# penn-graphics-research/HOT

Measured on AMD Instinct MI355X. Metric: ms per nonlinear (L-BFGS) iteration; P2G+G2P Mparticles/s; achieved HBM GB/s vs roofline, lower is better.
Workload: dtype f64; 1 GPU; C2: one 63^3-cell cube x 8 ppc (63^3 cells per GPU), fixed-corotated E=50000 nu=0.3, dx=0.01, dt=1/24, -lsolver 3 -mg_level 3 -smoother 5 -coarseSolver 2 --project --linesearch --bcproject --usecn -cneps 1e-7; particles_per_gpu=2000376, particles_total=2000376, nodes_total=267562, levels=3, parallelism=1 GPU

## Files before the change

### hot_amd/csrc/hot_common.h

```cpp
#pragma once
#include <hip/hip_runtime.h>
#include <cstdint>
#include <cstdio>
#include <cstring>
#include <cstdlib>
#include <string>
#include <vector>
#include <map>
#include <chrono>
#include "../../include/hot_mi355x.h"

namespace hot {

struct Error {
    int code;
    std::string msg;
};

#define HOT_HIP(expr)                                                                                             \
    do {                                                                                                          \
        hipError_t _e = (expr);                                                                                   \
        if (_e != hipSuccess) throw ::hot::Error{ HOT_ERR_DEVICE, std::string(#expr) + ": " + hipGetErrorString(_e) }; \
    } while (0)

// ... 109 lines not shown
    T d1 = d0 - (T)1;
    w[1] = (T)0.75 - d1 * d1;
    T d2 = (T)1 - d1;
    T zz = (T)1.5 - d2;
    w[2] = (T)0.5 * zz * zz;
    dw[0] = -z;
    dw[1] = -(T)2 * d1;
    dw[2] = zz;
}

template <int CTRL, int ROW_MASK>
__device__ __forceinline__ float dpp_move(float v)
{
    return __int_as_float(__builtin_amdgcn_update_dpp(0, __float_as_int(v), CTRL, ROW_MASK, 0xf, false));
}
template <int CTRL, int ROW_MASK>
__device__ __forceinline__ double dpp_move(double v)
{
    long long b = __double_as_longlong(v);
    int lo = __builtin_amdgcn_update_dpp(0, (int)(b & 0xffffffffLL), CTRL, ROW_MASK, 0xf, false);
    int hi = __builtin_amdgcn_update_dpp(0, (int)(b >> 32), CTRL, ROW_MASK, 0xf, false);
    return __longlong_as_double(((long long)hi << 32) | (unsigned int)lo);
}
__device__ __forceinline__ float wave_last(float v) { return __int_as_float(__builtin_amdgcn_readlane(__float_as_int(v), 63)); }
__device__ __forceinline__ double wave_last(double v)
{
    long long b = __double_as_longlong(v);
    int lo = __builtin_amdgcn_readlane((int)(b & 0xffffffffLL), 63), hi = __builtin_amdgcn_readlane((int)(b >> 32), 63);
    return __longlong_as_double(((long long)hi << 32) | (unsigned int)lo);
}
template <class T>
__device__ inline T wave_sum(T v)
{
    v += dpp_move<0xb1, 0xf>(v);
    v += dpp_move<0x4e, 0xf>(v);
    v += dpp_move<0x114, 0xf>(v);
    v += dpp_move<0x118, 0xf>(v);
    v += dpp_move<0x142, 0xa>(v);
    v += dpp_move<0x143, 0xc>(v);
    return wave_last(v);
}
template <class T>
__device__ inline T block_sum_256(T v, T* sm4)
{
    v = wave_sum(v);
    int lane = threadIdx.x & 63, w = threadIdx.x >> 6;
// ... 211 lines not shown
```

### hot_amd/csrc/mg_gs.hip

```cpp
#include "hot_impl.h"

namespace hot {

#ifdef HOT_AB_KERNELS
#include "ab_src/mg_gs_ab1.hip"
#endif

template <class T, int SB>
struct GsLds {
    static constexpr int TRI = SB * (SB - 1) / 2 + 1;
    static constexpr size_t bytes = (size_t)9 * TRI * sizeof(T) + SB * 3 * sizeof(T) + 5 * SB * sizeof(int32_t);
};
template <class T>
struct GsWinv {
    static constexpr int img_elems = (9 * GsLds<T, 64>::TRI + 15) / 16 * 16;
};
template <int SB>
__device__ __forceinline__ int gs_tri_fwd(int row, int colm) { return (SB - 1) * colm - (colm * (colm - 1)) / 2 + (row - colm - 1); }
__device__ __forceinline__ int gs_tri_bwd(int row, int colm) { return (colm * (colm - 1)) / 2 + row; }
template <bool FWD>
__device__ __forceinline__ int gs_winv_idx(int row, int colm) { return FWD ? (row * (row - 1)) / 2 + colm : ((63 - row) * (62 - row)) / 2 + (63 - colm); }

template <class T>
__device__ __forceinline__ void gs_store_tri(T* tri, int TRI, int idx, const T* __restrict__ di, const T (&b)[9])
// ... 678 lines not shown
__device__ unsigned long long gs_clk[34 * 8];
#define GS_CLK(i) \
    do { \
        const unsigned long long t_ = clock64(); \
        gclk_[i] += t_ - gt0_, gt0_ = t_; \
    } while (0)
#else
#define GS_CLK(i)
#endif
template <class T, bool FWD, int SB, bool WINV = false>
__global__ __launch_bounds__(SB * 16) void k_gs_sweep(const int32_t* __restrict__ col, const T* __restrict__ val, const uint32_t* __restrict__ ckey, const int32_t* __restrict__ gs_order,
    const int32_t* __restrict__ block_start, const T* __restrict__ diagVal, const T* __restrict__ diagBlockInv, const T* __restrict__ rhs, T* x, T* hD, GsPasses P,
    const int32_t* __restrict__ rowcnt, int* done, int* err, const int32_t* __restrict__ nbr, int* flag, int epoch, int dataflag,
    T* unset_next ,
    const T* __restrict__ gs_w )
{
    extern __shared__ __attribute__((aligned(16))) char gs_smem[];
    constexpr int TRI = GsLds<T, SB>::TRI;
    static_assert(!WINV || SB == 64, "the inverse images are whole-block images");
#ifdef HOT_GS_CLOCKS
    unsigned long long gclk_[5] = { 0, 0, 0, 0, 0 }, gt0_ = clock64();
#endif
    constexpr int RQ = 4, NW = SB / RQ;
    auto ld3 = [&](int64_t j, T& x0, T& x1, T& x2) {
        x0 = __hip_atomic_load(x + 3 * j, __ATOMIC_RELAXED, __HIP_MEMORY_SCOPE_AGENT), x1 = __hip_atomic_load(x + 3 * j + 1, __ATOMIC_RELAXED, __HIP_MEMORY_SCOPE_AGENT),
        x2 = __hip_atomic_load(x + 3 * j + 2, __ATOMIC_RELAXED, __HIP_MEMORY_SCOPE_AGENT);
        if (!dataflag) return;
        int spins = 0;
        while (GsUnset<T>::is(x0) || GsUnset<T>::is(x1) || GsUnset<T>::is(x2)) {
            __builtin_amdgcn_s_sleep(2);
            if (++spins > (1 << 21) || ((spins & 1023) == 0 && *(volatile int*)err)) {
                *(volatile int*)err = 1;
                break;
            }
            x0 = __hip_atomic_load(x + 3 * j, __ATOMIC_RELAXED, __HIP_MEMORY_SCOPE_AGENT), x1 = __hip_atomic_load(x + 3 * j + 1, __ATOMIC_RELAXED, __HIP_MEMORY_SCOPE_AGENT),
            x2 = __hip_atomic_load(x + 3 * j + 2, __ATOMIC_RELAXED, __HIP_MEMORY_SCOPE_AGENT);
        }
    };
    T* tri = (T*)gs_smem;
    T* sv = tri + (WINV ? GsWinv<T>::img_elems : 9 * TRI);
    int32_t* nodes = (int32_t*)(sv + 3 * SB);
    const int tid = threadIdx.x, lane = tid & 63, w = tid >> 6;
    int p = 0;
    while (p + 1 < P.npass && (int)blockIdx.x >= P.wg_begin[p + 1]) ++p;
    const int b = P.block0[p] + ((int)blockIdx.x - P.wg_begin[p]);
    const int lo = P.sub[p] * SB;
    const int start = block_start[b] + lo, cnt = max(0, min(SB, block_start[b + 1] - start));
    T* sDinv = (T*)(nodes + 5 * SB);
    T* sD = sDinv + 9 * SB;
    T* srhs = sD + 9 * SB;
    if (!WINV)
        for (int e = tid; e < 9 * TRI; e += 64 * NW) tri[e] = (T)0;
    if (tid < SB) nodes[tid] = tid < cnt ? gs_order[start + tid] : -1;
    __syncthreads();
    GS_CLK(0);
    if (WINV) {
        constexpr int IMG_BYTES = GsWinv<T>::img_elems * (int)sizeof(T);
        const char* wg = (const char*)(gs_w + ((size_t)b * 2 + (FWD ? 0 : 1)) * GsWinv<T>::img_elems);
        for (int c = w; c * 1024 < IMG_BYTES; c += NW) {
            const int off = c * 1024 + lane * 16;
            if (off < IMG_BYTES)
                __builtin_amdgcn_global_load_lds((const __attribute__((address_space(1))) void*)(wg + off), (__attribute__((address_space(3))) void*)((char*)tri + c * 1024), 16, 0, 0);
        }
    }
    for (int e = tid; e < 9 * cnt; e += 64 * NW) {
        const int64_t i = nodes[e / 9];
        sDinv[e] = diagBlockInv[9 * i + e % 9];
        if (FWD) sD[e] = diagVal[9 * i + e % 9];
    }
    for (int e = tid; e < 3 * cnt; e += 64 * NW) srhs[e] = rhs[3 * (int64_t)nodes[e / 3] + e % 3];
    if (unset_next)
        for (int e = tid; e < 3 * cnt; e += 64 * NW) gs_store_unset(unset_next + 3 * (int64_t)nodes[e / 3] + e % 3);
    T bv[RQ][9];
    int jj[RQ], node[RQ], kb2[RQ], ke[RQ];
    const bool first_sub = p == 0 || P.color[p - 1] != P.color[p];
    const bool head = FWD ? first_sub : !first_sub;
    bool late[RQ];
    const uint32_t prevkey = p > 0 ? ((uint32_t)P.color[p - 1] << 8) | (uint32_t)P.sub[p - 1] : 0xffffffffu;
    if constexpr (WINV) {
        int4 rc[RQ];
#pragma unroll
        for (int q = 0; q < RQ; ++q) {
            const int ii = w + NW * q;
            jj[q] = -1, kb2[q] = 0, ke[q] = 0, late[q] = false;
            node[q] = ii < cnt ? nodes[ii] : -1;
#pragma unroll
            for (int e = 0; e < 9; ++e) bv[q][e] = (T)0;
        }
#pragma unroll
        for (int q = 0; q < RQ; ++q) rc[q] = node[q] >= 0 ? *(const int4*)(rowcnt + 4 * (int64_t)node[q]) : make_int4(0, 0, 0, 0);
#pragma unroll
        for (int q = 0; q < RQ; ++q) {
            if (node[q] < 0) continue;
            const int64_t i = node[q];
            const int kbeg = FWD ? 0 : rc[q].x + rc[q].y + 1 + rc[q].z, kend = FWD ? rc[q].x : kbeg + rc[q].w;
            kb2[q] = head ? kbeg + 64 : kbeg, ke[q] = head ? kend : kend - 64;
            const int k = head ? kbeg + lane : kend - 64 + lane;
            if (k >= kbeg && k < kend) {
                jj[q] = col[i * 125 + k];
                const T* bb = val + (i * 125 + k) * 9;
#pragma unroll
                for (int e = 0; e < 9; ++e) bv[q][e] = bb[e];
            }
        }
#pragma unroll
        for (int q = 0; q < RQ; ++q)
            if (jj[q] >= 0) {
                const uint32_t keyj = ckey[jj[q]];
                late[q] = (((keyj >> 28) << 8) | (((keyj & 127u) - 1u) / (uint32_t)SB)) == prevkey;
            }
    }
    else
#pragma unroll
    for (int q = 0; q < RQ; ++q) {
        const int ii = w + NW * q;
        jj[q] = -1, node[q] = -1, kb2[q] = 0, ke[q] = 0, late[q] = false;
#pragma unroll
        for (int e = 0; e < 9; ++e) bv[q][e] = (T)0;
        if (ii < cnt) {
            const int i = nodes[ii];
            node[q] = i;
            const int po = rowcnt[4 * i], pi = rowcnt[4 * i + 1], fi = rowcnt[4 * i + 2], fo = rowcnt[4 * i + 3];
            const int kbeg = FWD ? 0 : po + pi + 1, kend = FWD ? po + pi : po + pi + 1 + fi + fo;
            const int ibeg = FWD ? po : kbeg, iend = FWD ? po + pi : kbeg + fi;
            kb2[q] = head ? kbeg + 64 : kbeg, ke[q] = head ? kend : kend - 64;
            const int k = head ? kbeg + lane : kend - 64 + lane;
            if (k >= kbeg && k < kend) {
                const int j = col[(int64_t)i * 125 + k];
                const T* bb = val + ((int64_t)i * 125 + k) * 9;
#pragma unroll
                for (int e = 0; e < 9; ++e) bv[q][e] = bb[e];
                jj[q] = j;
                const uint32_t keyj = ckey[j];
                late[q] = (((keyj >> 28) << 8) | (((keyj & 127u) - 1u) / (uint32_t)SB)) == prevkey;
                if (k >= ibeg && k < iend) {
                    const int l = (int)(keyj & 127u) - 1 - lo;
                    if (l >= 0 && l < SB) {
                        if (!WINV) {
                            const int idx = FWD ? gs_tri_fwd<SB>(ii, l) : gs_tri_bwd(ii, l);
                            gs_store_tri<T>(tri, TRI, idx, diagBlockInv + 9 * (int64_t)i, bv[q]);
                        }
                        jj[q] = -1;
                    }
                }
            }
        }
    }
    int early_idx = -1, late_idx = -1;
    if (nbr && tid < 26) {
        const int nb = nbr[(int64_t)b * 26 + tid];
        if (nb >= 0) {
            const int cn = nb >> 28, gid = nb & 0x0fffffff;
            int qlast = -1;
            for (int q = 0; q < P.npass; ++q)
                if (P.color[q] == cn) qlast = q;
            if (qlast >= 0 && qlast < p) {
                if (qlast < p - 1)
                    early_idx = 4 * gid + P.sub[qlast];
                else {
                    late_idx = 4 * gid + P.sub[qlast];
                    if (qlast > 0 && P.color[qlast - 1] == cn) early_idx = 4 * gid + P.sub[qlast - 1];
                }
            }
        }
    }
    if (nbr && tid == 26 && p > 0 && P.color[p - 1] == P.color[p]) late_idx = 4 * b + P.sub[p - 1];
    if (nbr && tid == 27 && p > 1 && P.color[p - 2] == P.color[p]) early_idx = 4 * b + P.sub[p - 2];
    auto wait_blocks = [&](int idx) {
        if (idx < 0) return;
        int spins = 0;
        while (__hip_atomic_load(flag + idx, __ATOMIC_RELAXED, __HIP_MEMORY_SCOPE_AGENT) != epoch) {
            __builtin_amdgcn_s_sleep(4);
            if (++spins > (1 << 22) || ((spins & 1023) == 0 && *(volatile int*)err)) {
                *(volatile int*)err = 1;
                break;
            }
        }
    };
    if (dataflag) {
    }
    else if (nbr)
        wait_blocks(early_idx);
    else if (p > 1 && tid == 0) {
        const int need2 = P.wg_begin[p - 1] - P.wg_begin[p - 2];
        int spins = 0;
        while (__hip_atomic_load(done + p - 2, __ATOMIC_RELAXED, __HIP_MEMORY_SCOPE_AGENT) < need2) {
            __builtin_amdgcn_s_sleep(4);
            if (++spins > (1 << 22) || ((spins & 1023) == 0 && *(volatile int*)err)) {
                *(volatile int*)err = 1;
                break;
            }
        }
    }
    __syncthreads();
    GS_CLK(1);
    auto is_late = [&](uint32_t keyj) { return (((keyj >> 28) << 8) | (((keyj & 127u) - 1u) / (uint32_t)SB)) == prevkey; };
    bool tail_late[RQ];
#pragma unroll
    for (int q = 0; q < RQ; ++q) {
        const int ii = w + NW * q;
        tail_late[q] = false;
        if (ii >= cnt) continue;
        const int i = node[q];
        T e0 = 0, e1 = 0, e2 = 0;
        if (jj[q] >= 0 && !late[q]) {
            const int64_t j = jj[q];
            T x0, x1, x2;
            ld3(j, x0, x1, x2);
            e0 = bv[q][0] * x0 + bv[q][3] * x1 + bv[q][6] * x2;
            e1 = bv[q][1] * x0 + bv[q][4] * x1 + bv[q][7] * x2;
            e2 = bv[q][2] * x0 + bv[q][5] * x1 + bv[q][8] * x2;
        }
        bool tl = false;
        for (int k = kb2[q] + lane; k < ke[q]; k += 64) {
            const int j = col[(int64_t)i * 125 + k];
            const T* bb = val + ((int64_t)i * 125 + k) * 9;
            const uint32_t keyj = ckey[j], keyi = ckey[i];
            const int l = (int)(keyj & 127u) - 1 - lo;
            if ((keyj >> 7) == (keyi >> 7) && l >= 0 && l < SB) {
                if (!WINV) {
                    const int idx = FWD ? gs_tri_fwd<SB>(ii, l) : gs_tri_bwd(ii, l);
                    T bt[9];
#pragma unroll
                    for (int e = 0; e < 9; ++e) bt[e] = bb[e];
                    gs_store_tri<T>(tri, TRI, idx, diagBlockInv + 9 * (int64_t)i, bt);
                }
            }
            else if (is_late(keyj))
                tl = true;
            else {
                T x0, x1, x2;
                ld3(j, x0, x1, x2);
                e0 += bb[0] * x0 + bb[3] * x1 + bb[6] * x2;
                e1 += bb[1] * x0 + bb[4] * x1 + bb[7] * x2;
                e2 += bb[2] * x0 + bb[5] * x1 + bb[8] * x2;
            }
        }
        tail_late[q] = __ballot(tl) != 0ull;
        e0 = wave_sum(e0), e1 = wave_sum(e1), e2 = wave_sum(e2);
        if (lane == 0) srhs[3 * ii] -= e0, srhs[3 * ii + 1] -= e1, srhs[3 * ii + 2] -= e2;
    }
    GS_CLK(2);
    if (!dataflag) {
        if (nbr)
            wait_blocks(late_idx);
        else if (p > 0 && tid == 0) {
            const int need = P.wg_begin[p] - P.wg_begin[p - 1];
            int spins = 0;
            while (__hip_atomic_load(done + p - 1, __ATOMIC_RELAXED, __HIP_MEMORY_SCOPE_AGENT) < need) {
                __builtin_amdgcn_s_sleep(4);
                ++spins;
                if ((spins & 1023) == 0 && *(volatile int*)err) break;
                if (spins > (1 << 22)) {
                    *(volatile int*)err = 1;
                    break;
                }
            }
        }
        __syncthreads();
    }
#pragma unroll
    for (int q = 0; q < RQ; ++q) {
        const int ii = w + NW * q;
        if (ii >= cnt) continue;
        const int i = node[q];
        T s0 = 0, s1 = 0, s2 = 0;
        if (jj[q] >= 0 && late[q]) {
            const int64_t j = jj[q];
            T x0, x1, x2;
            ld3(j, x0, x1, x2);
            s0 = bv[q][0] * x0 + bv[q][3] * x1 + bv[q][6] * x2;
            s1 = bv[q][1] * x0 + bv[q][4] * x1 + bv[q][7] * x2;
            s2 = bv[q][2] * x0 + bv[q][5] * x1 + bv[q][8] * x2;
        }
        if (tail_late[q]) {
            for (int k = kb2[q] + lane; k < ke[q]; k += 64) {
                const int j = col[(int64_t)i * 125 + k];
                const T* bb = val + ((int64_t)i * 125 + k) * 9;
                const uint32_t keyj = ckey[j], keyi = ckey[i];
                const int l = (int)(keyj & 127u) - 1 - lo;
                if (!((keyj >> 7) == (keyi >> 7) && l >= 0 && l < SB) && is_late(keyj)) {
                    T x0, x1, x2;
                    ld3(j, x0, x1, x2);
                    s0 += bb[0] * x0 + bb[3] * x1 + bb[6] * x2;
                    s1 += bb[1] * x0 + bb[4] * x1 + bb[7] * x2;
                    s2 += bb[2] * x0 + bb[5] * x1 + bb[8] * x2;
                }
            }
        }
        s0 = wave_sum(s0), s1 = wave_sum(s1), s2 = wave_sum(s2);
        if (lane == 0) gs_store_rhs<T>(sv, ii, sDinv + 9 * ii, srhs[3 * ii] - s0, srhs[3 * ii + 1] - s1, srhs[3 * ii + 2] - s2);
    }
    __syncthreads();
    GS_CLK(3);
#ifdef HOT_GS_CLOCKS
#define GS_CLK_OUT() \
    do { \
        GS_CLK(4); \
        if (tid == 0) \
// ... 19 lines not shown
            T t0 = Lw[0] * ac0 + Lw[3] * ac1 + Lw[6] * ac2, t1 = Lw[1] * ac0 + Lw[4] * ac1 + Lw[7] * ac2, t2 = Lw[2] * ac0 + Lw[5] * ac1 + Lw[8] * ac2;
            t0 = wave_sum(t0), t1 = wave_sum(t1), t2 = wave_sum(t2);
            if (lane == k) h0 = sv[3 * rr] + t0, h1 = sv[3 * rr + 1] + t1, h2 = sv[3 * rr + 2] + t2;
        }
        const int me = 4 * w + lane;
        if (lane < 4 && me < cnt) {
            const int64_t i = nodes[me];
            __hip_atomic_store(x + 3 * i, h0, __ATOMIC_RELAXED, __HIP_MEMORY_SCOPE_AGENT);
            __hip_atomic_store(x + 3 * i + 1, h1, __ATOMIC_RELAXED, __HIP_MEMORY_SCOPE_AGENT);
            __hip_atomic_store(x + 3 * i + 2, h2, __ATOMIC_RELAXED, __HIP_MEMORY_SCOPE_AGENT);
            if (FWD) {
                const T* dd = sD + 9 * me;
                hD[3 * i] = dd[0] * h0 + dd[3] * h1 + dd[6] * h2, hD[3 * i + 1] = dd[1] * h0 + dd[4] * h1 + dd[7] * h2, hD[3 * i + 2] = dd[2] * h0 + dd[5] * h1 + dd[8] * h2;
            }
            else if (hD)
                hD[3 * i] += h0, hD[3 * i + 1] += h1, hD[3 * i + 2] += h2;
        }
        GS_CLK_OUT();
        return;
    }
    if (w != 0) return;
    if (cnt > 0) gs_phase_b<T, FWD, SB, true>(tri, sv, nodes, cnt, lane, diagVal, diagBlockInv, x, hD, sD);
    GS_CLK_OUT();
    if (dataflag) return;
    asm volatile("s_waitcnt vmcnt(0)" ::: "memory");
    if (lane == 0) {
        if (nbr)
            __hip_atomic_store(flag + 4 * b + P.sub[p], epoch, __ATOMIC_RELAXED, __HIP_MEMORY_SCOPE_AGENT);
        else
            __hip_atomic_fetch_add(done + p, 1, __ATOMIC_RELAXED, __HIP_MEMORY_SCOPE_AGENT);
    }
}

template <class T>
__global__ void k_gs_hdiff(size_t n3, T* __restrict__ h, const T* __restrict__ du)
{
    const size_t i = (size_t)blockIdx.x * blockDim.x + threadIdx.x;
    if (i < n3) h[i] -= du[i];
}
template <class T, bool DIFF = false>
__global__ __launch_bounds__(256) void k_gs_residual(const int32_t* __restrict__ col, const T* __restrict__ val, const int32_t* __restrict__ rowcnt, const T* __restrict__ h,
    const T* __restrict__ du, T* __restrict__ r, int n, const uint8_t* __restrict__ own, const uint8_t* __restrict__ owner ,
    int me, const T* __restrict__ l1e )
{
    const int lane = threadIdx.x & 63;
    const int row = xcd_block() * 4 + (threadIdx.x >> 6);
    if (row >= n || (own && !own[row])) return;
// ... 335 lines not shown
        gs_done.reserve(64);
    }
    bool du_marked = false;
    auto chained_sweep = [&](bool fwd) {
        const GsPasses& P = fwd ? PF : PB;
        if (P.npass == 0) return;
        const char* nm = fwd ? "gs_forward" : "gs_backward";
        const T* rhs = fwd ? r : dAu;
        T* xx = fwd ? hdu : du;
        T* hD = fwd ? dAu : u;
        const int32_t* rc = L.rowcnt.p;
        const bool marked = fwd ? tmp_marked : du_marked;
        if (fwd) tmp_marked = false;
        if (plan.dataflag && !marked)
            HOT_LAUNCH(this, "gs_fill_unset", k_gs_fill_unset<T>, div_up(n3, 256), 256, 0, n3, xx);
        else if (plan.dataflag)
            ;
        else if (plan.p2p)
            ++gs_epoch;
        else
            HOT_HIP(hipMemsetAsync(gs_done.p, 0, 40 * sizeof(int), stream));
        const int grid = P.wg_begin[P.npass];
        const int dataflag = plan.dataflag ? 1 : 0;
#define HOT_GS_CASE(F, S, ...)                                                                                                                                         \
    HOT_LAUNCH(this, lname(nm, L.id).c_str(), (k_gs_sweep<T, F, S, ##__VA_ARGS__>), grid, 16 * S, (GsLds<T, S>::bytes + 21 * S * sizeof(T) + 128), L.col.p, L.val.p, L.ckey.p, L.gs_order.p, L.gs_block_start.p, \
        L.diagVal.p, L.diagBlockInv.p, rhs, xx, hD, P, rc, gs_done.p, (int*)(hscal + 250), plan.p2p ? L.gs_nbr.p : (const int32_t*)nullptr, L.gs_flag.p, gs_epoch, dataflag, \
        (fwd && dataflag) ? du : (T*)nullptr, L.gs_w.p)
        du_marked = fwd && dataflag;
        if (plan.winv) {
            if (fwd)
                HOT_GS_CASE(true, 64, true);
            else
                HOT_GS_CASE(false, 64, true);
        }
        else if (fwd) {
            if (sb == 64) HOT_GS_CASE(true, 64);
            else if (sb == 32) HOT_GS_CASE(true, 32);
            else HOT_GS_CASE(true, 16);
        }
        else {
            if (sb == 64) HOT_GS_CASE(false, 64);
            else if (sb == 32) HOT_GS_CASE(false, 32);
            else HOT_GS_CASE(false, 16);
        }
#undef HOT_GS_CASE
    };
// ... 83 lines not shown
```

### hot_amd/csrc/mg_solve.hip

```cpp
#include "hot_impl.h"
#include "hot_svd.h"

namespace hot {

template <class T>
__global__ void k_axpy(size_t n, T a, const T* __restrict__ x, T* y)
{
    size_t i = (size_t)blockIdx.x * blockDim.x + threadIdx.x;
    if (i < n) y[i] += a * x[i];
}
template <class T>
__global__ void k_axpy_dev(size_t n, const double* a, double sign, const T* __restrict__ x, T* y)
{
    size_t i = (size_t)blockIdx.x * blockDim.x + threadIdx.x;
    T s = (T)(sign * (*a));
    if (i < n) y[i] += s * x[i];
}
template <class T>
__global__ void k_xpay_dev(size_t n, const double* a, const T* __restrict__ x, T* y)
{
    size_t i = (size_t)blockIdx.x * blockDim.x + threadIdx.x;
    T s = (T)(*a);
    if (i < n) y[i] = x[i] + s * y[i];
}
// ... 200 lines not shown
template <class T>
__global__ void k_cg_direction(size_t n3, const T* __restrict__ z, T* __restrict__ du, double* s, double* hm, double* ticket, double ticket_val)
{
    const size_t i = (size_t)blockIdx.x * blockDim.x + threadIdx.x;
    const bool act = cg_active(s[0], s[8]);
    if (act && i < n3) du[i] = z[i] + (T)(s[4] / s[0]) * du[i];
    if (i == 0) {
        if (act) {
            s[6] = 1.0;
            const double cnt = s[9] + 1.0;
            s[9] = cnt;
            hm[0] = s[4], hm[1] = cnt;
        }
        if (ticket) host_ticket_store(ticket, ticket_val);
    }
}
template <class T, int RPW = 0>
__global__ __launch_bounds__(1024) void k_cg_persist(const int32_t* __restrict__ col, const T* __restrict__ val, const T* __restrict__ Dinv, const T* __restrict__ init, T* __restrict__ u,
    T* __restrict__ r, T* __restrict__ z, T* du, T* __restrict__ dAu, int n, int max_iters, unsigned phase0 , double* dep , int SS , double* hm, double* ticket, double ticket_val,
    int* err )
{
    __shared__ double red[32], sres[2];
    __shared__ int s_bail;
    const int tid = threadIdx.x, lane = tid & 63, w = tid >> 6;
    const int G = gridDim.x, wg = blockIdx.x;
    unsigned phase = phase0;
    if (tid == 0) s_bail = 0;
    auto ldu = [&](int64_t j, int c) { return __hip_atomic_load(du + 3 * j + c, __ATOMIC_RELAXED, __HIP_MEMORY_SCOPE_AGENT); };
    auto sdu = [&](int64_t j, int c, T v) { __hip_atomic_store(du + 3 * j + c, v, __ATOMIC_RELAXED, __HIP_MEMORY_SCOPE_AGENT); };
    auto all_sum = [&](double v0, double v1, double& o0, double& o1) -> bool {
        asm volatile("s_waitcnt vmcnt(0)" ::: "memory");
        if (lane == 0) red[w] = v0, red[16 + w] = v1;
        __syncthreads();
        double* d = dep + (size_t)(phase & 3u) * G * SS;
        if (tid == 0) {
            double t0 = 0, t1 = 0;
            for (int k = 0; k < 16; ++k) t0 += red[k], t1 += red[16 + k];
            double* dn = dep + (size_t)((phase + 2u) & 3u) * G * SS + (size_t)wg * SS;
            __hip_atomic_store((unsigned long long*)dn, GsUnset<double>::bits, __ATOMIC_RELAXED, __HIP_MEMORY_SCOPE_AGENT);
            __hip_atomic_store((unsigned long long*)(dn + 1), GsUnset<double>::bits, __ATOMIC_RELAXED, __HIP_MEMORY_SCOPE_AGENT);
            __hip_atomic_store(d + (size_t)wg * SS, t0, __ATOMIC_RELAXED, __HIP_MEMORY_SCOPE_AGENT);
            __hip_atomic_store(d + (size_t)wg * SS + 1, t1, __ATOMIC_RELAXED, __HIP_MEMORY_SCOPE_AGENT);
        }
        if (w < 2) {
            const double* dv = d + w;
            double a = 0;
            int spins = 0, bail = 0;
// ... 1 lines not shown
                bool all = true;
                a = 0;
                for (int k = lane; k < G; k += 64) {
                    const double x = __hip_atomic_load(dv + (size_t)k * SS, __ATOMIC_RELAXED, __HIP_MEMORY_SCOPE_AGENT);
                    all = all && !GsUnset<double>::is(x);
                    a += x;
                }
                if (__all(all)) break;
                __builtin_amdgcn_s_sleep(1);
                if (++spins > (1 << 21) || ((spins & 255) == 0 && *(volatile int*)err)) {
                    *(volatile int*)err = 1;
                    bail = 1;
                    break;
                }
            }
            a = wave_sum(a);
            if (lane == 0) {
                sres[w] = a;
                if (bail) s_bail = 1;
            }
        }
        __syncthreads();
        if (s_bail) return false;
        o0 = sres[0], o1 = sres[1];
        ++phase;
        return true;
    };
    auto scale = [&](int64_t i, const T (&v)[3], T (&o)[3]) {
        const T* d = Dinv + 9 * i;
        o[0] = d[0] * v[0] + d[3] * v[1] + d[6] * v[2], o[1] = d[1] * v[0] + d[4] * v[1] + d[7] * v[2], o[2] = d[2] * v[0] + d[5] * v[1] + d[8] * v[2];
    };
    const int stride = 16 * G;
    if constexpr (RPW > 0) {
        int rowq[RPW];
        int32_t mc[RPW][2];
        T mv[RPW][2][9], di[RPW][9], uu[RPW][3], rr[RPW][3], zz[RPW][3], dd[RPW][3], ad[RPW][3];
        double p0 = 0, p1 = 0;
#pragma unroll
        for (int q = 0; q < RPW; ++q) {
            const int row = wg * 16 + w + q * stride;
            rowq[q] = row < n ? row : -1;
            const int64_t rc = row < n ? row : 0;
#pragma unroll
            for (int h = 0; h < 2; ++h) {
                const int k = min(lane + 64 * h, 124);
                mc[q][h] = col[rc * 125 + k];
#pragma unroll
                for (int e = 0; e < 9; ++e) mv[q][h][e] = (lane + 64 * h < 125) ? val[rc * 1125 + k * 9 + e] : (T)0;
            }
#pragma unroll
            for (int e = 0; e < 9; ++e) di[q][e] = Dinv[9 * rc + e];
            T a[3], za[3];
#pragma unroll
            for (int c = 0; c < 3; ++c) a[c] = init[3 * rc + c], rr[q][c] = r[3 * rc + c], uu[q][c] = u[3 * rc + c], ad[q][c] = (T)0;
#pragma unroll
            for (int c = 0; c < 3; ++c) za[c] = di[q][c] * a[0] + di[q][3 + c] * a[1] + di[q][6 + c] * a[2], zz[q][c] = di[q][c] * rr[q][0] + di[q][3 + c] * rr[q][1] + di[q][6 + c] * rr[q][2];
            if (lane == 0 && rowq[q] >= 0) {
                p0 += (double)(za[0] * a[0]) + (double)(za[1] * a[1]) + (double)(za[2] * a[2]);
                p1 += (double)(zz[q][0] * rr[q][0]) + (double)(zz[q][1] * rr[q][1]) + (double)(zz[q][2] * rr[q][2]);
                for (int c = 0; c < 3; ++c) sdu(row, c, zz[q][c]);
            }
#pragma unroll
            for (int c = 0; c < 3; ++c) dd[q][c] = zz[q][c];
        }
        double zTr0, zTr;
        if (!all_sum(p0, p1, zTr0, zTr)) return;
        const double tol = (double)(T)(zTr0 * 0.25);
        extern __shared__ double cg_lds[];
        T* ldsdu = (T*)cg_lds;
        const int n3 = 3 * n;
        auto pull_du = [&]() {
            const int n16 = n3 >> 1;
            for (int e0 = 0; e0 < n16; e0 += 4 * 1024) {
                double2 v[4];
#pragma unroll
                for (int k = 0; k < 4; ++k) {
                    const int e = min(e0 + k * 1024 + tid, n16 - 1);
                    asm volatile("global_load_dwordx4 %0, %1, off sc0 sc1" : "=v"(v[k]) : "v"((const double2*)du + e) : "memory");
                }
                asm volatile("s_waitcnt vmcnt(0)" ::: "memory");
#pragma unroll
                for (int k = 0; k < 4; ++k) {
                    const int e = e0 + k * 1024 + tid;
                    if (e < n16) ((double2*)ldsdu)[e] = v[k];
                }
            }
            if ((n3 & 1) && tid == 0) ldsdu[n3 - 1] = ldu(n - 1, 2);
            __syncthreads();
        };
        int cnt = 0;
#ifdef HOT_AB_KERNELS
        unsigned long long tk[8] = { 0, 0, 0, 0, 0, 0, 0, 0 }, t0_ = wall_clock64();
#define CG_TK(i) \
    do { \
        const unsigned long long t_ = wall_clock64(); \
        tk[i] += t_ - t0_, t0_ = t_; \
    } while (0)
#else
#define CG_TK(i)
#endif
        for (; cnt < max_iters && cg_active(zTr, tol); ++cnt) {
            pull_du();
            CG_TK(0);
            double pd = 0;
#pragma unroll
            for (int q = 0; q < RPW; ++q) {
                T s0 = 0, s1 = 0, s2 = 0;
#pragma unroll
                for (int h = 0; h < 2; ++h) {
                    if (lane + 64 * h < 125) {
                        const int j = mc[q][h];
                        const T* b = mv[q][h];
                        const T x0 = ldsdu[3 * j], x1 = ldsdu[3 * j + 1], x2 = ldsdu[3 * j + 2];
                        s0 += b[0] * x0 + b[3] * x1 + b[6] * x2;
                        s1 += b[1] * x0 + b[4] * x1 + b[7] * x2;
                        s2 += b[2] * x0 + b[5] * x1 + b[8] * x2;
                    }
                }
                s0 = wave_sum(s0), s1 = wave_sum(s1), s2 = wave_sum(s2);
                ad[q][0] = s0, ad[q][1] = s1, ad[q][2] = s2;
                if (lane == 0 && rowq[q] >= 0) pd += (double)(s0 * dd[q][0]) + (double)(s1 * dd[q][1]) + (double)(s2 * dd[q][2]);
            }
            CG_TK(1);
            double dAd, unused;
            if (!all_sum(pd, 0.0, dAd, unused)) return;
            CG_TK(2);
            const double omega = zTr / dAd;
            const T wp = (T)omega, wm = (T)(-omega);
            double pz = 0;
#pragma unroll
            for (int q = 0; q < RPW; ++q) {
#pragma unroll
                for (int c = 0; c < 3; ++c) uu[q][c] += wp * dd[q][c], rr[q][c] = rr[q][c] + wm * ad[q][c];
#pragma unroll
                for (int c = 0; c < 3; ++c) zz[q][c] = di[q][c] * rr[q][0] + di[q][3 + c] * rr[q][1] + di[q][6 + c] * rr[q][2];
                if (lane == 0 && rowq[q] >= 0) pz += (double)(zz[q][0] * rr[q][0]) + (double)(zz[q][1] * rr[q][1]) + (double)(zz[q][2] * rr[q][2]);
            }
            CG_TK(3);
            double zTrNew;
            if (!all_sum(pz, 0.0, zTrNew, unused)) return;
            CG_TK(4);
            const T beta = (T)(zTrNew / zTr);
#pragma unroll
            for (int q = 0; q < RPW; ++q) {
#pragma unroll
                for (int c = 0; c < 3; ++c) dd[q][c] = zz[q][c] + beta * dd[q][c];
                if (lane == 0 && rowq[q] >= 0)
                    for (int c = 0; c < 3; ++c) sdu(rowq[q], c, dd[q][c]);
            }
            zTr = zTrNew;
            CG_TK(5);
            if (!all_sum(0.0, 0.0, unused, unused)) return;
            CG_TK(6);
        }
#ifdef HOT_AB_KERNELS
        if (tid == 0 && wg == 0)
            for (int i = 0; i < 7; ++i) hm[8 + i] = (double)tk[i];
#endif
#pragma unroll
        for (int q = 0; q < RPW; ++q)
            if (lane == 0 && rowq[q] >= 0)
                for (int c = 0; c < 3; ++c) {
                    const int64_t e = 3 * (int64_t)rowq[q] + c;
                    u[e] = uu[q][c], r[e] = rr[q][c], z[e] = zz[q][c], dAu[e] = ad[q][c];
                }
        if (tid == 0 && wg == 0) {
            hm[0] = zTr, hm[1] = (double)cnt, hm[2] = tol;
            if (ticket) host_ticket_store(ticket, ticket_val);
        }
        return;
    }
    double p0 = 0, p1 = 0;
    for (int row = wg * 16 + w; row < n; row += stride) {
        if (lane == 0) {
            T a[3] = { init[3 * (int64_t)row], init[3 * (int64_t)row + 1], init[3 * (int64_t)row + 2] }, za[3];
            scale(row, a, za);
            p0 += (double)(za[0] * a[0]) + (double)(za[1] * a[1]) + (double)(za[2] * a[2]);
            T b[3] = { r[3 * (int64_t)row], r[3 * (int64_t)row + 1], r[3 * (int64_t)row + 2] }, zb[3];
            scale(row, b, zb);
            for (int c = 0; c < 3; ++c) z[3 * (int64_t)row + c] = zb[c], sdu(row, c, zb[c]);
            p1 += (double)(zb[0] * b[0]) + (double)(zb[1] * b[1]) + (double)(zb[2] * b[2]);
        }
    }
    double zTr0, zTr;
    if (!all_sum(p0, p1, zTr0, zTr)) return;
    const double tol = (double)(T)(zTr0 * 0.25);
    int cnt = 0;
    for (; cnt < max_iters && cg_active(zTr, tol); ++cnt) {
        double pd = 0;
        for (int row = wg * 16 + w; row < n; row += stride) {
// ... 27 lines not shown
            if (lane == 0) {
                T rr[3], zz[3];
                for (int c = 0; c < 3; ++c) {
                    u[3 * (int64_t)row + c] += wp * ldu(row, c);
                    rr[c] = r[3 * (int64_t)row + c] + wm * dAu[3 * (int64_t)row + c];
                    r[3 * (int64_t)row + c] = rr[c];
                }
                scale(row, rr, zz);
                for (int c = 0; c < 3; ++c) z[3 * (int64_t)row + c] = zz[c];
                pz += (double)(zz[0] * rr[0]) + (double)(zz[1] * rr[1]) + (double)(zz[2] * rr[2]);
            }
        }
        double zTrNew;
        if (!all_sum(pz, 0.0, zTrNew, unused)) return;
        const T beta = (T)(zTrNew / zTr);
        for (int row = wg * 16 + w; row < n; row += stride)
            if (lane == 0)
                for (int c = 0; c < 3; ++c) sdu(row, c, z[3 * (int64_t)row + c] + beta * ldu(row, c));
        zTr = zTrNew;
        if (!all_sum(0.0, 0.0, unused, unused)) return;
    }
    if (tid == 0) {
        if (wg == 0) {
            hm[0] = zTr, hm[1] = (double)cnt, hm[2] = tol;
            if (ticket) host_ticket_store(ticket, ticket_val);
        }
    }
}

template <class T>
__global__ void k_scal_v(size_t n, T a, T* x)
{
    size_t i = (size_t)blockIdx.x * blockDim.x + threadIdx.x;
    if (i < n) x[i] *= a;
}
template <class T>
void Ctx<T>::scal(size_t n, T a, T* x)
{
    HOT_LAUNCH(this, "scal", k_scal_v<T>, div_up(n, 256), 256, 0, n, a, x);
}
template <class T>
void Ctx<T>::spmv_dev(Level<T>& L, const T* x, T* y)
{
    if (L.part && halo_mode()) halo_gather(L, const_cast<T*>(x));
    HOT_LAUNCH(this, lname("spmv", L.id).c_str(), k_spmv<T>, xcd_grid(div_up(L.n, 4)), 256, 0, L.col.p, L.val.p, x, y, L.n, L.mask());
    if (!halo_mode()) exchange(L, y, -1);
}
// ... 208 lines not shown
            const int cg_ss = ab_int("HOT_CG_SLOT_STRIDE", 32);
            if (!cg_dep.p || cg_bar_dirty || cg_G != G) {
                cg_dep.reserve((size_t)4 * 256 * cg_ss);
                HOT_LAUNCH(this, "gs_fill_unset", k_gs_fill_unset<double>, div_up((size_t)4 * 256 * cg_ss, 256), 256, 0, (size_t)4 * 256 * cg_ss, cg_dep.p);
                cg_bar_dirty = false, cg_G = G, cg_phase = 0;
            }
            const bool cg_resident = L.n <= 2 * 16 * G && 3 * (size_t)L.n * sizeof(double) <= 150 * 1024 && !ab_flag("HOT_CG_STREAM");
            if (cg_resident && !attr_cg_set) {
                HOT_HIP(hipFuncSetAttribute((const void*)k_cg_persist<T, 2>, hipFuncAttributeMaxDynamicSharedMemorySize, 150 * 1024));
                attr_cg_set = true;
            }
            if (cg_resident)
                HOT_LAUNCH(this, lname("cg_persistent", L.id).c_str(), (k_cg_persist<T, 2>), G, 1024, 3 * (size_t)L.n * sizeof(double), L.col.p, L.val.p, L.diagInv.p, L.initialResidual.p, u, r, z, du, dAu, L.n, iterations, cg_phase, cg_dep.p, cg_ss,
                    hscal + 40, hscal + 251, new_ticket(), (int*)(hscal + 250));
            else
                HOT_LAUNCH(this, lname("cg_persistent", L.id).c_str(), k_cg_persist<T>, G, 1024, 0, L.col.p, L.val.p, L.diagInv.p, L.initialResidual.p, u, r, z, du, dAu, L.n, iterations, cg_phase, cg_dep.p, cg_ss,
                    hscal + 40, hscal + 251, new_ticket(), (int*)(hscal + 250));
            wait_ticket();
            cnt = (int)hscal[41];
            if (ab_flag("HOT_CG_DBG"))
                fprintf(stderr, "cg_persistent level %d: %d rows, %d workgroups, %d iterations; ticks pull %.0f product %.0f barrier1 %.0f update %.0f barrier2 %.0f direction %.0f barrier3 %.0f\n", L.id, L.n, G, cnt,
                    hscal[48], hscal[49], hscal[50], hscal[51], hscal[52], hscal[53], hscal[54]);
            cg_phase = (cg_phase + 1u + 3u * (unsigned)cnt) & 3u;
            iterations = 0;
        }
        else if (fused) {
            scaler(L.initialResidual.p, z);
            dot_to(n3, z, L.initialResidual.p, s + 7);
            scaler(r, z);
            copy(n3, z, du);
            dot_to(n3, z, r, s);
            HOT_LAUNCH(this, "cg_setup", k_cg_setup<T>, 1, 1, 0, s, hscal + 40);
            int group = std::max(1, std::min(cg_group, 16));
            bool active = true;
            while (iterations > 0 && active) {
                const int g = std::min(group, iterations);
                for (int k = 0; k < g; ++k) {
                    HOT_LAUNCH(this, lname("spmv", L.id).c_str(), k_cg_spmv_dot<T>, div_up(L.n, 4), 256, 0, L.col.p, L.val.p, du, dAu, L.n, s, gred(div_up(L.n, 4)));
                    HOT_LAUNCH(this, "cg_update", k_cg_update<T>, div_up(L.n, 256), 256, 0, L.diagInv.p, du, dAu, u, r, z, L.n, s, gred(div_up(L.n, 256)));
                    const bool last = k + 1 == g;
                    HOT_LAUNCH(this, "cg_direction", k_cg_direction<T>, div_up(n3, 256), 256, 0, n3, z, du, s, hscal + 40, last ? hscal + 251 : (double*)nullptr, last ? new_ticket() : 0.0);
                }
                iterations -= g;
                wait_ticket();
                active = !(hscal[40] < hscal[42]);
                group = 2;
// ... 212 lines not shown
```

Baseline: 3.256 ms/iter.

## Cut register pressure in GS sweep and persistent CG by moving per-row state to LDS

In the resident persistent CG kernel, the per-row CG state (Dinv, u, r, z, d, Ad) moves from per-lane register arrays into a shared-memory table that only lane 0 updates. The wave index and reduction results are made wave-uniform, and du loads use a scalar base address. The aim is to lower VGPR use and raise occupancy, at the cost of extra LDS traffic. In the GS sweep, the non-A/B build hardwires the data-flag spin path, stores each row's column range in LDS, and reloads the late block from global memory instead of holding it in registers. The change also adds a host phase-consistency check and a kernel-resource inspection script.

```diff
diff --git a/hot_amd/csrc/hot_common.h b/hot_amd/csrc/hot_common.h
--- a/hot_amd/csrc/hot_common.h
+++ b/hot_amd/csrc/hot_common.h
@@ -155,6 +155,12 @@
     int hi = __builtin_amdgcn_update_dpp(0, (int)(b >> 32), CTRL, ROW_MASK, 0xf, false);
     return __longlong_as_double(((long long)hi << 32) | (unsigned int)lo);
 }
+__device__ __forceinline__ double wave_first(double v)
+{
+    long long b = __double_as_longlong(v);
+    int lo = __builtin_amdgcn_readfirstlane((int)(b & 0xffffffffLL)), hi = __builtin_amdgcn_readfirstlane((int)(b >> 32));
+    return __longlong_as_double(((long long)hi << 32) | (unsigned int)lo);
+}
 __device__ __forceinline__ float wave_last(float v) { return __int_as_float(__builtin_amdgcn_readlane(__float_as_int(v), 63)); }
 __device__ __forceinline__ double wave_last(double v)
 {
diff --git a/hot_amd/csrc/mg_gs.hip b/hot_amd/csrc/mg_gs.hip
--- a/hot_amd/csrc/mg_gs.hip
+++ b/hot_amd/csrc/mg_gs.hip
@@ -724,10 +724,15 @@
     unsigned long long gclk_[5] = { 0, 0, 0, 0, 0 }, gt0_ = clock64();
 #endif
     constexpr int RQ = 4, NW = SB / RQ;
+#ifdef HOT_AB_KERNELS
+    const bool dflag = WINV || dataflag != 0;
+#else
+    constexpr bool dflag = true;
+#endif
     auto ld3 = [&](int64_t j, T& x0, T& x1, T& x2) {
         x0 = __hip_atomic_load(x + 3 * j, __ATOMIC_RELAXED, __HIP_MEMORY_SCOPE_AGENT), x1 = __hip_atomic_load(x + 3 * j + 1, __ATOMIC_RELAXED, __HIP_MEMORY_SCOPE_AGENT),
         x2 = __hip_atomic_load(x + 3 * j + 2, __ATOMIC_RELAXED, __HIP_MEMORY_SCOPE_AGENT);
-        if (!dataflag) return;
+        if (!dflag) return;
         int spins = 0;
         while (GsUnset<T>::is(x0) || GsUnset<T>::is(x1) || GsUnset<T>::is(x2)) {
             __builtin_amdgcn_s_sleep(2);
@@ -748,6 +753,7 @@
     const int b = P.block0[p] + ((int)blockIdx.x - P.wg_begin[p]);
     const int lo = P.sub[p] * SB;
     const int start = block_start[b] + lo, cnt = max(0, min(SB, block_start[b + 1] - start));
+    int32_t* rng = nodes + SB;
     T* sDinv = (T*)(nodes + 5 * SB);
     T* sD = sDinv + 9 * SB;
     T* srhs = sD + 9 * SB;
@@ -785,7 +791,7 @@
         for (int q = 0; q < RQ; ++q) {
             const int ii = w + NW * q;
             jj[q] = -1, kb2[q] = 0, ke[q] = 0, late[q] = false;
-            node[q] = ii < cnt ? nodes[ii] : -1;
+            node[q] = ii < cnt ? __builtin_amdgcn_readfirstlane(nodes[ii]) : -1;
 #pragma unroll
             for (int e = 0; e < 9; ++e) bv[q][e] = (T)0;
         }
@@ -826,6 +832,7 @@
             const int kbeg = FWD ? 0 : po + pi + 1, kend = FWD ? po + pi : po + pi + 1 + fi + fo;
             const int ibeg = FWD ? po : kbeg, iend = FWD ? po + pi : kbeg + fi;
             kb2[q] = head ? kbeg + 64 : kbeg, ke[q] = head ? kend : kend - 64;
+            rng[ii] = kb2[q], rng[SB + ii] = ke[q];
             const int k = head ? kbeg + lane : kend - 64 + lane;
             if (k >= kbeg && k < kend) {
                 const int j = col[(int64_t)i * 125 + k];
@@ -849,7 +856,7 @@
         }
     }
     int early_idx = -1, late_idx = -1;
-    if (nbr && tid < 26) {
+    if (!dflag && nbr && tid < 26) {
         const int nb = nbr[(int64_t)b * 26 + tid];
         if (nb >= 0) {
             const int cn = nb >> 28, gid = nb & 0x0fffffff;
@@ -866,8 +873,8 @@
             }
         }
     }
-    if (nbr && tid == 26 && p > 0 && P.color[p - 1] == P.color[p]) late_idx = 4 * b + P.sub[p - 1];
-    if (nbr && tid == 27 && p > 1 && P.color[p - 2] == P.color[p]) early_idx = 4 * b + P.sub[p - 2];
+    if (!dflag && nbr && tid == 26 && p > 0 && P.color[p - 1] == P.color[p]) late_idx = 4 * b + P.sub[p - 1];
+    if (!dflag && nbr && tid == 27 && p > 1 && P.color[p - 2] == P.color[p]) early_idx = 4 * b + P.sub[p - 2];
     auto wait_blocks = [&](int idx) {
         if (idx < 0) return;
         int spins = 0;
@@ -879,7 +886,7 @@
             }
         }
     };
-    if (dataflag) {
+    if (dflag) {
     }
     else if (nbr)
         wait_blocks(early_idx);
@@ -903,7 +910,7 @@
         const int ii = w + NW * q;
         tail_late[q] = false;
         if (ii >= cnt) continue;
-        const int i = node[q];
+        const int i = WINV ? node[q] : nodes[ii], kt0 = WINV ? kb2[q] : rng[ii], kt1 = WINV ? ke[q] : rng[SB + ii];
         T e0 = 0, e1 = 0, e2 = 0;
         if (jj[q] >= 0 && !late[q]) {
             const int64_t j = jj[q];
@@ -914,7 +921,7 @@
             e2 = bv[q][2] * x0 + bv[q][5] * x1 + bv[q][8] * x2;
         }
         bool tl = false;
-        for (int k = kb2[q] + lane; k < ke[q]; k += 64) {
+        for (int k = kt0 + lane; k < kt1; k += 64) {
             const int j = col[(int64_t)i * 125 + k];
             const T* bb = val + ((int64_t)i * 125 + k) * 9;
             const uint32_t keyj = ckey[j], keyi = ckey[i];
@@ -943,7 +950,7 @@
         if (lane == 0) srhs[3 * ii] -= e0, srhs[3 * ii + 1] -= e1, srhs[3 * ii + 2] -= e2;
     }
     GS_CLK(2);
-    if (!dataflag) {
+    if (!dflag) {
         if (nbr)
             wait_blocks(late_idx);
         else if (p > 0 && tid == 0) {
@@ -961,22 +968,28 @@
         }
         __syncthreads();
     }
+    const T* val_again = val;
+    asm volatile("" : "+s"(val_again));
 #pragma unroll
     for (int q = 0; q < RQ; ++q) {
         const int ii = w + NW * q;
         if (ii >= cnt) continue;
-        const int i = node[q];
+        const int i = WINV ? node[q] : nodes[ii], kt0 = WINV ? kb2[q] : rng[ii], kt1 = WINV ? ke[q] : rng[SB + ii];
         T s0 = 0, s1 = 0, s2 = 0;
         if (jj[q] >= 0 && late[q]) {
             const int64_t j = jj[q];
+            const T* bb = val_again + ((int64_t)i * 125 + (head ? kt0 - 64 : kt1) + lane) * 9;
+            T bl[9];
+#pragma unroll
+            for (int e = 0; e < 9; ++e) bl[e] = bb[e];
             T x0, x1, x2;
             ld3(j, x0, x1, x2);
-            s0 = bv[q][0] * x0 + bv[q][3] * x1 + bv[q][6] * x2;
-            s1 = bv[q][1] * x0 + bv[q][4] * x1 + bv[q][7] * x2;
-            s2 = bv[q][2] * x0 + bv[q][5] * x1 + bv[q][8] * x2;
+            s0 = bl[0] * x0 + bl[3] * x1 + bl[6] * x2;
+            s1 = bl[1] * x0 + bl[4] * x1 + bl[7] * x2;
+            s2 = bl[2] * x0 + bl[5] * x1 + bl[8] * x2;
         }
         if (tail_late[q]) {
-            for (int k = kb2[q] + lane; k < ke[q]; k += 64) {
+            for (int k = kt0 + lane; k < kt1; k += 64) {
                 const int j = col[(int64_t)i * 125 + k];
                 const T* bb = val + ((int64_t)i * 125 + k) * 9;
                 const uint32_t keyj = ckey[j], keyi = ckey[i];
@@ -1042,7 +1055,7 @@
     if (w != 0) return;
     if (cnt > 0) gs_phase_b<T, FWD, SB, true>(tri, sv, nodes, cnt, lane, diagVal, diagBlockInv, x, hD, sD);
     GS_CLK_OUT();
-    if (dataflag) return;
+    if (dflag) return;
     asm volatile("s_waitcnt vmcnt(0)" ::: "memory");
     if (lane == 0) {
         if (nbr)
@@ -1424,6 +1437,9 @@
             HOT_HIP(hipMemsetAsync(gs_done.p, 0, 40 * sizeof(int), stream));
         const int grid = P.wg_begin[P.npass];
         const int dataflag = plan.dataflag ? 1 : 0;
+#ifndef HOT_AB_KERNELS
+        HOT_CHECK(dataflag, HOT_ERR_INVALID, "k_gs_sweep: only the A/B build carries the stamp and pass-counter hand-offs");
+#endif
 #define HOT_GS_CASE(F, S, ...)                                                                                                                                         \
     HOT_LAUNCH(this, lname(nm, L.id).c_str(), (k_gs_sweep<T, F, S, ##__VA_ARGS__>), grid, 16 * S, (GsLds<T, S>::bytes + 21 * S * sizeof(T) + 128), L.col.p, L.val.p, L.ckey.p, L.gs_order.p, L.gs_block_start.p, \
         L.diagVal.p, L.diagBlockInv.p, rhs, xx, hD, P, rc, gs_done.p, (int*)(hscal + 250), plan.p2p ? L.gs_nbr.p : (const int32_t*)nullptr, L.gs_flag.p, gs_epoch, dataflag, \
diff --git a/hot_amd/csrc/mg_solve.hip b/hot_amd/csrc/mg_solve.hip
--- a/hot_amd/csrc/mg_solve.hip
+++ b/hot_amd/csrc/mg_solve.hip
@@ -246,7 +246,9 @@
 {
     __shared__ double red[32], sres[2];
     __shared__ int s_bail;
-    const int tid = threadIdx.x, lane = tid & 63, w = tid >> 6;
+    enum { CG_DI = 0, CG_U = 9, CG_R = 12, CG_Z = 15, CG_D = 18, CG_AD = 21 };
+    __shared__ T cg_row[RPW > 0 ? 16 : 1][RPW > 0 ? RPW : 1][24];
+    const int tid = threadIdx.x, lane = tid & 63, w = __builtin_amdgcn_readfirstlane(tid >> 6);
     const int G = gridDim.x, wg = blockIdx.x;
     unsigned phase = phase0;
     if (tid == 0) s_bail = 0;
@@ -294,7 +296,7 @@
         }
         __syncthreads();
         if (s_bail) return false;
-        o0 = sres[0], o1 = sres[1];
+        o0 = wave_first(sres[0]), o1 = wave_first(sres[1]);
         ++phase;
         return true;
     };
@@ -306,7 +308,7 @@
     if constexpr (RPW > 0) {
         int rowq[RPW];
         int32_t mc[RPW][2];
-        T mv[RPW][2][9], di[RPW][9], uu[RPW][3], rr[RPW][3], zz[RPW][3], dd[RPW][3], ad[RPW][3];
+        T mv[RPW][2][9];
         double p0 = 0, p1 = 0;
 #pragma unroll
         for (int q = 0; q < RPW; ++q) {
@@ -320,20 +322,23 @@
 #pragma unroll
                 for (int e = 0; e < 9; ++e) mv[q][h][e] = (lane + 64 * h < 125) ? val[rc * 1125 + k * 9 + e] : (T)0;
             }
-#pragma unroll
-            for (int e = 0; e < 9; ++e) di[q][e] = Dinv[9 * rc + e];
-            T a[3], za[3];
-#pragma unroll
-            for (int c = 0; c < 3; ++c) a[c] = init[3 * rc + c], rr[q][c] = r[3 * rc + c], uu[q][c] = u[3 * rc + c], ad[q][c] = (T)0;
-#pragma unroll
-            for (int c = 0; c < 3; ++c) za[c] = di[q][c] * a[0] + di[q][3 + c] * a[1] + di[q][6 + c] * a[2], zz[q][c] = di[q][c] * rr[q][0] + di[q][3 + c] * rr[q][1] + di[q][6 + c] * rr[q][2];
-            if (lane == 0 && rowq[q] >= 0) {
-                p0 += (double)(za[0] * a[0]) + (double)(za[1] * a[1]) + (double)(za[2] * a[2]);
-                p1 += (double)(zz[q][0] * rr[q][0]) + (double)(zz[q][1] * rr[q][1]) + (double)(zz[q][2] * rr[q][2]);
-                for (int c = 0; c < 3; ++c) sdu(row, c, zz[q][c]);
-            }
-#pragma unroll
-            for (int c = 0; c < 3; ++c) dd[q][c] = zz[q][c];
+            if (lane == 0) {
+                T* st = cg_row[w][q];
+                T di[9], a[3], za[3], rr[3], zz[3];
+#pragma unroll
+                for (int e = 0; e < 9; ++e) di[e] = Dinv[9 * rc + e], st[CG_DI + e] = di[e];
+#pragma unroll
+                for (int c = 0; c < 3; ++c) a[c] = init[3 * rc + c], rr[c] = r[3 * rc + c], st[CG_U + c] = u[3 * rc + c], st[CG_AD + c] = (T)0;
+#pragma unroll
+                for (int c = 0; c < 3; ++c) za[c] = di[c] * a[0] + di[3 + c] * a[1] + di[6 + c] * a[2], zz[c] = di[c] * rr[0] + di[3 + c] * rr[1] + di[6 + c] * rr[2];
+                if (rowq[q] >= 0) {
+                    p0 += (double)(za[0] * a[0]) + (double)(za[1] * a[1]) + (double)(za[2] * a[2]);
+                    p1 += (double)(zz[0] * rr[0]) + (double)(zz[1] * rr[1]) + (double)(zz[2] * rr[2]);
+                    for (int c = 0; c < 3; ++c) sdu(row, c, zz[c]);
+                }
+#pragma unroll
+                for (int c = 0; c < 3; ++c) st[CG_R + c] = rr[c], st[CG_Z + c] = zz[c], st[CG_D + c] = zz[c];
+            }
         }
         double zTr0, zTr;
         if (!all_sum(p0, p1, zTr0, zTr)) return;
@@ -347,8 +352,8 @@
                 double2 v[4];
 #pragma unroll
                 for (int k = 0; k < 4; ++k) {
-                    const int e = min(e0 + k * 1024 + tid, n16 - 1);
-                    asm volatile("global_load_dwordx4 %0, %1, off sc0 sc1" : "=v"(v[k]) : "v"((const double2*)du + e) : "memory");
+                    const unsigned eb = 16u * (unsigned)min(e0 + k * 1024 + tid, n16 - 1);
+                    asm volatile("global_load_dwordx4 %0, %1, %2 sc0 sc1" : "=v"(v[k]) : "v"(eb), "s"(du) : "memory");
                 }
                 asm volatile("s_waitcnt vmcnt(0)" ::: "memory");
 #pragma unroll
@@ -390,8 +395,11 @@
                     }
                 }
                 s0 = wave_sum(s0), s1 = wave_sum(s1), s2 = wave_sum(s2);
-                ad[q][0] = s0, ad[q][1] = s1, ad[q][2] = s2;
-                if (lane == 0 && rowq[q] >= 0) pd += (double)(s0 * dd[q][0]) + (double)(s1 * dd[q][1]) + (double)(s2 * dd[q][2]);
+                if (lane == 0) {
+                    T* st = cg_row[w][q];
+                    st[CG_AD] = s0, st[CG_AD + 1] = s1, st[CG_AD + 2] = s2;
+                    if (rowq[q] >= 0) pd += (double)(s0 * st[CG_D]) + (double)(s1 * st[CG_D + 1]) + (double)(s2 * st[CG_D + 2]);
+                }
             }
             CG_TK(1);
             double dAd, unused;
@@ -400,25 +408,35 @@
             const double omega = zTr / dAd;
             const T wp = (T)omega, wm = (T)(-omega);
             double pz = 0;
-#pragma unroll
-            for (int q = 0; q < RPW; ++q) {
-#pragma unroll
-                for (int c = 0; c < 3; ++c) uu[q][c] += wp * dd[q][c], rr[q][c] = rr[q][c] + wm * ad[q][c];
-#pragma unroll
-                for (int c = 0; c < 3; ++c) zz[q][c] = di[q][c] * rr[q][0] + di[q][3 + c] * rr[q][1] + di[q][6 + c] * rr[q][2];
-                if (lane == 0 && rowq[q] >= 0) pz += (double)(zz[q][0] * rr[q][0]) + (double)(zz[q][1] * rr[q][1]) + (double)(zz[q][2] * rr[q][2]);
+            if (lane == 0) {
+#pragma unroll
+                for (int q = 0; q < RPW; ++q) {
+                    T* st = cg_row[w][q];
+                    T rr[3], zz[3];
+#pragma unroll
+                    for (int c = 0; c < 3; ++c) st[CG_U + c] += wp * st[CG_D + c], rr[c] = st[CG_R + c] + wm * st[CG_AD + c];
+#pragma unroll
+                    for (int c = 0; c < 3; ++c) zz[c] = st[CG_DI + c] * rr[0] + st[CG_DI + 3 + c] * rr[1] + st[CG_DI + 6 + c] * rr[2];
+                    if (rowq[q] >= 0) pz += (double)(zz[0] * rr[0]) + (double)(zz[1] * rr[1]) + (double)(zz[2] * rr[2]);
+#pragma unroll
+                    for (int c = 0; c < 3; ++c) st[CG_R + c] = rr[c], st[CG_Z + c] = zz[c];
+                }
             }
             CG_TK(3);
             double zTrNew;
             if (!all_sum(pz, 0.0, zTrNew, unused)) return;
             CG_TK(4);
             const T beta = (T)(zTrNew / zTr);
-#pragma unroll
-            for (int q = 0; q < RPW; ++q) {
-#pragma unroll
-                for (int c = 0; c < 3; ++c) dd[q][c] = zz[q][c] + beta * dd[q][c];
-                if (lane == 0 && rowq[q] >= 0)
-                    for (int c = 0; c < 3; ++c) sdu(rowq[q], c, dd[q][c]);
+            if (lane == 0) {
+#pragma unroll
+                for (int q = 0; q < RPW; ++q) {
+                    T* st = cg_row[w][q];
+                    T dd[3];
+#pragma unroll
+                    for (int c = 0; c < 3; ++c) dd[c] = st[CG_Z + c] + beta * st[CG_D + c], st[CG_D + c] = dd[c];
+                    if (rowq[q] >= 0)
+                        for (int c = 0; c < 3; ++c) sdu(rowq[q], c, dd[c]);
+                }
             }
             zTr = zTrNew;
             CG_TK(5);
@@ -431,13 +449,15 @@
 #endif
 #pragma unroll
         for (int q = 0; q < RPW; ++q)
-            if (lane == 0 && rowq[q] >= 0)
+            if (lane == 0 && rowq[q] >= 0) {
+                const T* st = cg_row[w][q];
                 for (int c = 0; c < 3; ++c) {
                     const int64_t e = 3 * (int64_t)rowq[q] + c;
-                    u[e] = uu[q][c], r[e] = rr[q][c], z[e] = zz[q][c], dAu[e] = ad[q][c];
-                }
+                    u[e] = st[CG_U + c], r[e] = st[CG_R + c], z[e] = st[CG_Z + c], dAu[e] = st[CG_AD + c];
+                }
+            }
         if (tid == 0 && wg == 0) {
-            hm[0] = zTr, hm[1] = (double)cnt, hm[2] = tol;
+            hm[0] = zTr, hm[1] = (double)cnt, hm[2] = tol, hm[3] = (double)(phase & 3u);
             if (ticket) host_ticket_store(ticket, ticket_val);
         }
         return;
@@ -511,7 +531,7 @@
     }
     if (tid == 0) {
         if (wg == 0) {
-            hm[0] = zTr, hm[1] = (double)cnt, hm[2] = tol;
+            hm[0] = zTr, hm[1] = (double)cnt, hm[2] = tol, hm[3] = (double)(phase & 3u);
             if (ticket) host_ticket_store(ticket, ticket_val);
         }
     }
@@ -766,6 +786,7 @@
                 fprintf(stderr, "cg_persistent level %d: %d rows, %d workgroups, %d iterations; ticks pull %.0f product %.0f barrier1 %.0f update %.0f barrier2 %.0f direction %.0f barrier3 %.0f\n", L.id, L.n, G, cnt,
                     hscal[48], hscal[49], hscal[50], hscal[51], hscal[52], hscal[53], hscal[54]);
             cg_phase = (cg_phase + 1u + 3u * (unsigned)cnt) & 3u;
+            HOT_CHECK((unsigned)hscal[43] == cg_phase, HOT_ERR_DEVICE, "k_cg_persist passed another number of barriers than the host counts: the next launch would start on the wrong set of deposit slots");
             iterations = 0;
         }
         else if (fused) {
diff --git a/hot_amd/kernel_resources.py b/hot_amd/kernel_resources.py
--- /dev/null
+++ b/hot_amd/kernel_resources.py
@@ -0,0 +1,78 @@
+import os
+import re
+import shutil
+import subprocess
+import tempfile
+
+LLVM_BIN = os.path.join(os.environ.get("ROCM_PATH", "/opt/rocm"), "lib", "llvm", "bin")
+OBJDUMP = os.path.join(LLVM_BIN, "llvm-objdump")
+READELF = os.path.join(LLVM_BIN, "llvm-readelf")
+TARGET = "hipv4-amdgcn-amd-amdhsa--gfx950"
+
+_FIELDS = {
+    "agpr": "agpr_count", "vgpr": "vgpr_count", "sgpr": "sgpr_count", "vgpr_spill": "vgpr_spill_count", "sgpr_spill": "sgpr_spill_count",
+    "scratch": "private_segment_fixed_size", "lds": "group_segment_fixed_size", "max_threads": "max_flat_workgroup_size",
+}
+_BUILTIN = {"d": "double", "f": "float", "i": "int", "j": "unsigned", "b": "bool", "h": "unsigned char", "t": "unsigned short", "l": "long", "m": "unsigned long"}
+
+
+def tools_missing():
+    for t in (OBJDUMP, READELF):
+        if not os.path.exists(t):
+            return t
+    return None
+
+
+def short_name(symbol):
+    m = re.match(r"_ZN3hot(\d+)", symbol)
+    if not m:
+        return symbol
+    n, at = int(m.group(1)), m.end()
+    name, rest = symbol[at:at + n], symbol[at + n:]
+    if not rest.startswith("I"):
+        return "hot::" + name
+    args, i = [], 1
+    while i < len(rest) and rest[i] != "E":
+        if rest[i] in _BUILTIN:
+            args.append(_BUILTIN[rest[i]])
+            i += 1
+            continue
+        lit = re.match(r"L([a-z])(n?)(\d+)E", rest[i:])
+        if not lit:
+            return symbol
+        ty, neg, val = lit.groups()
+        args.append(("true" if val != "0" else "false") if ty == "b" else ("-" if neg else "") + val)
+        i += lit.end()
+    return "hot::%s<%s>" % (name, ", ".join(args))
+
+
+def waves_per_simd(vgpr, agpr=0):
+    alloc = max(8, -(-(vgpr + agpr) // 8) * 8)
+    return min(8, 512 // alloc)
+
+
+def read(lib_path):
+    out = {}
+    with tempfile.TemporaryDirectory() as tmp:
+        copy = os.path.join(tmp, "lib.so")
+        shutil.copy(lib_path, copy)
+        subprocess.run([OBJDUMP, "--offloading", copy], check=True, cwd=tmp, stdout=subprocess.DEVNULL, stderr=subprocess.DEVNULL)
+        images = sorted(f for f in os.listdir(tmp) if f.endswith(TARGET))
+        if not images:
+            raise RuntimeError("%s holds no %s image" % (lib_path, TARGET))
+        for img in images:
+            notes = subprocess.run([READELF, "--notes", os.path.join(tmp, img)], check=True, capture_output=True, text=True).stdout
+            for blk in re.split(r"^\s*- (?=\.agpr_count:)", notes, flags=re.M)[1:]:
+                sym = re.search(r"^\s*\.symbol:\s+(\S+)", blk, flags=re.M)
+                if not sym:
+                    continue
+                k = {"symbol": sym.group(1)[:-3] if sym.group(1).endswith(".kd") else sym.group(1)}
+                for key, field in _FIELDS.items():
+                    m = re.search(r"^\s*\.%s:\s+(\d+)" % field, blk, flags=re.M)
+                    k[key] = int(m.group(1)) if m else 0
+                k["name"] = short_name(k["symbol"])
+                k["waves_per_simd"] = waves_per_simd(k["vgpr"], k["agpr"])
+                prev = out.get(k["symbol"])
+                if prev is None or (k["scratch"], k["vgpr_spill"], k["vgpr"]) > (prev["scratch"], prev["vgpr_spill"], prev["vgpr"]):
+                    out[k["symbol"]] = k
+    return sorted(out.values(), key=lambda k: k["name"])
```

After: 3.079 ms/iter (median of 6 runs). 1.06x faster.
